# nv-tlabs/LION

Measured on AMD Instinct MI355X. Metric: shapes/sec @1000-step DDIM, Bx2048pts, higher is better.
Workload: dtype f32 (operands of the 3x3x3 voxel convolutions and of the long 1x1 convolutions cut into fp16 hi/lo pairs on the 16-bi...

## Files before the change

### lion_amd/csrc/pwconv_split.hip

```cpp
#include "split_ops.h"

namespace {

#ifdef PWS_TIMING
__device__ unsigned long long g_pws_t[128];
#define PWS_T(i) do { if (tid == 0 && blockIdx.x == 0 && blockIdx.y == 0 && blockIdx.z == 0 && (i) < 128) g_pws_t[i] = __builtin_readcyclecounter(); } while (0)
#else
#define PWS_T(i) do { } while (0)
#endif

template <int CB, int VB, bool PRO, bool STATS, int NR>
__global__ __launch_bounds__(256, 2) void pwconv_split_kernel(const float *__restrict__ x, const u4 *__restrict__ wp,
                                                           const float *__restrict__ wtail,
                                                           const float *__restrict__ bias, float *__restrict__ y,
                                                           int Cin, int Cpad, int CoutY, int L,
                                                           const float *__restrict__ pro_a,
                                                           const float *__restrict__ pro_b, float *__restrict__ stats) {
  constexpr int COT = 32 * CB, WPL = 4 * COT;
  constexpr int NDMA = WPL / 64, DMIN = NDMA / 4;
  extern __shared__ __attribute__((aligned(16))) unsigned char smem[];
  constexpr int D = NR - 1;
  u4 *sw = reinterpret_cast<u4 *>(smem);
  const int nchunks = (Cin + KS - 1) / KS;
  constexpr int RING_U4 = NR * WPL > 4 * 32 * 9 ? NR * WPL : 4 * 32 * 9;
  float *spa = reinterpret_cast<float *>(sw + RING_U4);
  float *spb = spa + (PRO ? nchunks * KS : 0);
  float *sbias = spb + (PRO ? nchunks * KS : 0);
  float *sred = sbias + COT;
  const int tid = threadIdx.x, lane = tid & 63, wave = __builtin_amdgcn_readfirstlane(tid >> 6);
  const int l32 = lane & 31, kh = lane >> 5;
  const int b = blockIdx.z, co0 = blockIdx.y * COT;
  PWS_T(0);
  if (PRO) {
    for (int c = tid; c < nchunks * KS; c += 256) {
      spa[c] = c < Cin ? pro_a[(size_t)b * Cin + c] : 0.f;
      spb[c] = c < Cin ? pro_b[(size_t)b * Cin + c] : 0.f;
    }
  }
  if (tid < COT) sbias[tid] = (bias && co0 + tid < CoutY) ? bias[co0 + tid] : 0.f;
  int colc[VB];
  bool cok[VB];
#pragma unroll
  for (int vb = 0; vb < VB; ++vb) {
    const int col = ((blockIdx.x * 4 + wave) * VB + vb) * 32 + l32;
    cok[vb] = col < L;
    colc[vb] = cok[vb] ? col : L - 1;
  }
  const __amdgpu_buffer_rsrc_t xrs = __builtin_amdgcn_make_buffer_rsrc(
      const_cast<float *>(x + (size_t)b * Cin * L), 0, Cin * L * 4, 0x00020000);
  typedef __attribute__((address_space(3))) unsigned char lds_byte;
  const uint32_t sw_lds = (uint32_t)(uintptr_t)(lds_byte *)reinterpret_cast<unsigned char *>(sw);
  auto weights_dma = [&](int q) {
    if (q >= nchunks) return;
    const uint32_t dst0 = sw_lds + (uint32_t)((q % NR) * WPL * 16);
    for (int i = wave; i < NDMA; i += 4) {
      const int e = i * 64 + lane;
      const u4 *gp = wp + ((size_t)q * 4 + e / COT) * Cpad + co0 + e % COT;
      const uint32_t dst = __builtin_amdgcn_readfirstlane(dst0 + (uint32_t)(i * 1024));
      unsigned keep;
      asm volatile("s_mov_b32 %0, m0\n\ts_mov_b32 m0, %2\n\ts_nop 0\n\tglobal_load_lds_dwordx4 %1, off\n\ts_mov_b32 m0, %0"
                   : "=&s"(keep) : "v"(gp), "s"(dst) : "memory");
    }
  };
  auto issue_x = [&](int q, float (&v)[VB][8]) {
#pragma unroll
    for (int vb = 0; vb < VB; ++vb) {
      const int off0 = ((q * KS + kh * 8) * L + colc[vb]) * 4;
#pragma unroll
      for (int j = 0; j < 8; ++j)
        v[vb][j] = __builtin_bit_cast(float, __builtin_amdgcn_raw_buffer_load_b32(xrs, off0 + j * L * 4, 0, 0));
    }
  };
  f32x16 acc[CB][VB], cor[CB][VB];
#pragma unroll
  for (int cb = 0; cb < CB; ++cb)
#pragma unroll
    for (int vb = 0; vb < VB; ++vb)
#pragma unroll
      for (int i = 0; i < 16; ++i) acc[cb][vb][i] = cor[cb][vb][i] = 0.f;
  int E[VB];
#pragma unroll
  for (int vb = 0; vb < VB; ++vb) E[vb] = 127;

  auto chunk = [&](int q, float (&v)[VB][8], float (&vnext)[VB][8]) {
    static_assert((D - 1) * (DMIN + 8 * VB) <= 63, "vmcnt is a 6-bit counter");
    const int behind = max(0, min(D - 1, nchunks - 1 - q));
    if (behind >= 3 && D > 3) wait_vm<(D - 1) * 8 * VB + (D > 3 ? 3 : 0) * DMIN>();
    else if (behind == 2 && D > 2) wait_vm<(D - 1) * 8 * VB + (D > 2 ? 2 : 0) * DMIN>();
    else if (behind == 1 && D > 1) wait_vm<(D - 1) * 8 * VB + DMIN>();
    else wait_vm<(D - 1) * 8 * VB>();
    PWS_T(2 + 4 * q);
    __syncthreads();
    PWS_T(3 + 4 * q);
    weights_dma(q + D);
    issue_x(q + D, vnext);
    PWS_T(4 + 4 * q);
    if (q >= nchunks) return;
    const u4 *swq = sw + (q % NR) * WPL;
    u4 wh[CB], wl[CB];
#pragma unroll
    for (int cb = 0; cb < CB; ++cb) { wh[cb] = swq[(0 + kh) * COT + cb * 32 + l32]; wl[cb] = swq[(2 + kh) * COT + cb * 32 + l32]; }
    u4 xh[VB], xl[VB];
#pragma unroll
    for (int vb = 0; vb < VB; ++vb) {
      float t[8];
      unsigned m = 0u;
      float pa[8], pb[8];
      if (PRO) {
        const float4 a0 = *reinterpret_cast<const float4 *>(spa + q * KS + kh * 8), a1 = *reinterpret_cast<const float4 *>(spa + q * KS + kh * 8 + 4);
        const float4 b0 = *reinterpret_cast<const float4 *>(spb + q * KS + kh * 8), b1 = *reinterpret_cast<const float4 *>(spb + q * KS + kh * 8 + 4);
        pa[0] = a0.x; pa[1] = a0.y; pa[2] = a0.z; pa[3] = a0.w; pa[4] = a1.x; pa[5] = a1.y; pa[6] = a1.z; pa[7] = a1.w;
        pb[0] = b0.x; pb[1] = b0.y; pb[2] = b0.z; pb[3] = b0.w; pb[4] = b1.x; pb[5] = b1.y; pb[6] = b1.z; pb[7] = b1.w;
      }
#pragma unroll
      for (int j = 0; j < 8; ++j) {
        float u = v[vb][j];
        if (PRO) u = pro_act(u, pa[j], pb[j]);
        u = (q * KS + kh * 8 + j < Cin && cok[vb]) ? u : 0.f;
        t[j] = u;
        const unsigned a = __float_as_uint(u) & 0x7fffffffu;
        m = (a > m && a <= 0x7f7fffffu) ? a : m;
      }
      const unsigned mo = __shfl_xor(m, 32, 64);
      m = mo > m ? mo : m;
      if (m) {
        const int e = scale_exp(__uint_as_float(m));
        if (e < E[vb]) {
          if (E[vb] != 127) {
            const float f = pow2f(max(e - PW_SPLIT_HEADROOM - E[vb], -126));
#pragma unroll
            for (int cb = 0; cb < CB; ++cb)
#pragma unroll
              for (int i = 0; i < 16; ++i) { acc[cb][vb][i] *= f; cor[cb][vb][i] *= f; }
          }
          E[vb] = e - PW_SPLIT_HEADROOM;
        }
      }
      const float xs = E[vb] == 127 ? 1.0f : pow2f(E[vb]);
#pragma unroll
      for (int k = 0; k < 4; ++k) { unsigned h2, l2; cut2(t[2 * k] * xs, t[2 * k + 1] * xs, h2, l2); xh[vb][k] = h2; xl[vb][k] = l2; }
    }
    PWS_T(64 + q);
#pragma unroll
    for (int cb = 0; cb < CB; ++cb)
#pragma unroll
      for (int vb = 0; vb < VB; ++vb) acc[cb][vb] = mma(wh[cb], xh[vb], acc[cb][vb]);
#pragma unroll
    for (int cb = 0; cb < CB; ++cb)
#pragma unroll
      for (int vb = 0; vb < VB; ++vb) cor[cb][vb] = mma(wh[cb], xl[vb], cor[cb][vb]);
#pragma unroll
    for (int cb = 0; cb < CB; ++cb)
#pragma unroll
      for (int vb = 0; vb < VB; ++vb) cor[cb][vb] = mma(wl[cb], xh[vb], cor[cb][vb]);
    PWS_T(5 + 4 * q);
  };

  static_assert(D >= 1 && D <= 4, "the wait above distinguishes up to 3 chunks in flight behind the awaited one");
  float ring[NR][VB][8];
#pragma unroll
  for (int p = 0; p < D; ++p) { weights_dma(p); issue_x(p, ring[p]); }
  PWS_T(1);
  for (int q0 = 0; q0 < nchunks; q0 += NR) {
#pragma unroll
    for (int p = 0; p < NR; ++p)
      chunk(q0 + p, ring[p], ring[(p + D) % NR]);
  }

  PWS_T(100);
  const float us_w = wtail[2];
  float *yb = y + ((size_t)b * CoutY + co0) * L;
  const bool full = co0 + COT <= CoutY;
#pragma unroll
  for (int vb = 0; vb < VB; ++vb) {
    const float us_x = E[vb] == 127 ? 1.0f : pow2f(-E[vb]);
#pragma unroll
    for (int cb = 0; cb < CB; ++cb)
#pragma unroll
      for (int i = 0; i < 16; ++i) {
        const int co = cb * 32 + (i & 3) + 8 * (i >> 2) + 4 * kh;
        const float o = ((acc[cb][vb][i] + cor[cb][vb][i] * (1.f / 2048.f)) * us_x) * us_w + sbias[co];
        acc[cb][vb][i] = cok[vb] ? o : 0.f;
      }
    float *yc = yb + colc[vb];
    if (full) {
      if (cok[vb]) {
#pragma unroll
        for (int cb = 0; cb < CB; ++cb)
#pragma unroll
          for (int i = 0; i < 16; ++i) yc[(size_t)(cb * 32 + (i & 3) + 8 * (i >> 2) + 4 * kh) * L] = acc[cb][vb][i];
      }
    } else {
#pragma unroll
      for (int cb = 0; cb < CB; ++cb)
#pragma unroll
        for (int i = 0; i < 16; ++i) {
          const int co = cb * 32 + (i & 3) + 8 * (i >> 2) + 4 * kh;
          if (cok[vb] && co0 + co < CoutY) yc[(size_t)co * L] = acc[cb][vb][i];
        }
    }
  }
  PWS_T(102);
  if (STATS) {
    __syncthreads();
    float *T = reinterpret_cast<float *>(sw) + wave * (32 * 36);
    const int hc = lane >> 5;
#pragma unroll
    for (int cb = 0; cb < CB; ++cb) {
      float s1 = 0.f, s2 = 0.f;
#pragma unroll
      for (int vb = 0; vb < VB; ++vb) {
#pragma unroll
        for (int i = 0; i < 16; ++i) T[((i & 3) + 8 * (i >> 2) + 4 * kh) * 36 + l32] = acc[cb][vb][i];
        __builtin_amdgcn_fence(__ATOMIC_RELEASE, "wavefront");
        __builtin_amdgcn_wave_barrier();
        __builtin_amdgcn_fence(__ATOMIC_ACQUIRE, "wavefront");
#pragma unroll
        for (int j = 0; j < 4; ++j) {
          const float4 t = *reinterpret_cast<const float4 *>(T + l32 * 36 + hc * 16 + 4 * j);
          s1 += t.x; s2 += t.x * t.x;
          s1 += t.y; s2 += t.y * t.y;
          s1 += t.z; s2 += t.z * t.z;
          s1 += t.w; s2 += t.w * t.w;
        }
        __builtin_amdgcn_fence(__ATOMIC_RELEASE, "wavefront");
        __builtin_amdgcn_wave_barrier();
      }
      sred[((wave * 2 + hc) * COT + cb * 32 + l32) * 2] = s1;
      sred[((wave * 2 + hc) * COT + cb * 32 + l32) * 2 + 1] = s2;
    }
    PWS_T(103);
    __syncthreads();
    for (int c = tid; c < COT && co0 + c < CoutY; c += 256) {
      float s1 = 0.f, s2 = 0.f;
#pragma unroll
      for (int w = 0; w < 8; ++w) { s1 += sred[(w * COT + c) * 2]; s2 += sred[(w * COT + c) * 2 + 1]; }
      float *o = stats + (((size_t)b * CoutY + co0 + c) * gridDim.x + blockIdx.x) * 2;
      o[0] = s1;
      o[1] = s2;
    }
  }
  PWS_T(101);
}

template <bool TR>
__global__ void pw_split_pack_kernel(const float *__restrict__ w, int Cout, int Cpad, int Cin, int nchunks,
                                     unsigned short *__restrict__ wp, unsigned *__restrict__ tail,
                                     const unsigned *__restrict__ tail_src) {
  const int i = blockIdx.x * blockDim.x + threadIdx.x;
  int ew;
  if (TR) {
    ew = (int)tail_src[1];
    if (i < 4) tail[i] = tail_src[i];
  } else {
    ew = split_tail_scale(tail, i == 0);
  }
  if (i >= nchunks * KS * Cpad) return;
  const int co = i % Cpad, k = i / Cpad, q = k / KS, g = (k % KS) / 8, j = k % 8;
  unsigned short hi = 0, lo = 0;
  if (co < Cout && k < Cin) cut((TR ? w[(size_t)k * Cout + co] : w[(size_t)co * Cin + k]) * pow2f(ew), hi, lo);
  const size_t base = (size_t)q * 4;
  wp[((base + 0 + g) * Cpad + co) * 8 + j] = hi;
  wp[((base + 2 + g) * Cpad + co) * 8 + j] = lo;
}

#ifndef PWS_NR
#define PWS_NR 5
#endif
struct PwSplitPlan { int cb, vb; };
static int pws_pad(int Cout) { return (Cout + 31) / 32 * 32; }
static PwSplitPlan pws_plan(int Cout) {
  const int blocks = pws_pad(Cout) / 32;
  if (blocks <= 0) return {0, 0};
  if (blocks % 4 == 0) return {4, 1};
  if (blocks % 2 == 0) return {2, 2};
  return {1, 2};
}
static size_t pws_halfs(int Cout, int Cin) { return (size_t)((Cin + KS - 1) / KS) * 4 * pws_pad(Cout) * 8; }

template <int CB, int VB, int NR>
static int launch_pws(const float *x, const u4 *wp, const float *wtail, const float *bias, float *y, int B, int Cin,
                      int Cout, int L, const float *pa, const float *pb, float *stats, hipStream_t st) {
  const int Cpad = pws_pad(Cout), nchunks = (Cin + KS - 1) / KS;
  const dim3 grid(lion_cdiv(L, 4 * VB * 32), Cpad / (CB * 32), B);
  const size_t ring = (size_t)NR * 4 * CB * 32 * 16, tile = (size_t)4 * 32 * 36 * 4;
  const size_t lds = (ring > tile ? ring : tile) + (size_t)((pa ? 2 * nchunks * KS : 0) + CB * 32 + 8 * CB * 32 * 2) * 4;
#define LION_PWS_GO(PRO_, ST_)                                                                             \
  {                                                                                                        \
    static LionLdsLimit cfg = {};                                                                          \
    if (int e = lion_dynamic_lds(&pwconv_split_kernel<CB, VB, PRO_, ST_, NR>, lds, cfg)) return e;             \
    pwconv_split_kernel<CB, VB, PRO_, ST_, NR><<<grid, 256, lds, st>>>(x, wp, wtail, bias, y, Cin, Cpad, Cout, L, pa, pb, stats); \
  }
  if (pa && stats) LION_PWS_GO(true, true)
  else if (pa) LION_PWS_GO(true, false)
  else if (stats) LION_PWS_GO(false, true)
  else LION_PWS_GO(false, false)
#undef LION_PWS_GO
  LION_LAUNCH_CHECK();
  return 0;
}

}

extern "C" {

#ifdef PWS_TIMING
int lion_debug_pws_times(unsigned long long *host128) {
  return hipMemcpyFromSymbol(host128, HIP_SYMBOL(g_pws_t), 1024) == hipSuccess ? 0 : -1;
}
#endif

size_t lion_pwconv_split_packed_halfs(int Cout, int Cin) { return pws_halfs(Cout, Cin) + 8; }

int lion_pwconv_split_pack_weights(const float *w, int Cout, int Cin, uint16_t *wp, lionStream_t stream) {
  if (!w || !wp || Cout <= 0 || Cin <= 0) return LION_EINVAL;
  if ((((uintptr_t)wp) & 15) != 0) return LION_EUNSUPPORTED;
  hipStream_t st = static_cast<hipStream_t>(stream);
  unsigned *tail = reinterpret_cast<unsigned *>(wp + pws_halfs(Cout, Cin));
  const int n = Cout * Cin, nchunks = (Cin + KS - 1) / KS, Cpad = pws_pad(Cout);
  if (hipMemsetAsync(tail, 0, 16, st) != hipSuccess) return LION_EINVAL;
  split_wmax_kernel<<<min(lion_cdiv(n, 2048), 128), 256, 0, st>>>(w, n, tail);
  pw_split_pack_kernel<false><<<lion_cdiv(nchunks * KS * Cpad, 256), 256, 0, st>>>(w, Cout, Cpad, Cin, nchunks, wp, tail, nullptr);
  LION_LAUNCH_CHECK();
  return 0;
}

int lion_pwconv_split_pack_weights_t(const float *w, int Cout, int Cin, const uint16_t *wp, uint16_t *wpt, lionStream_t stream) {
  if (!w || !wp || !wpt || Cout <= 0 || Cin <= 0) return LION_EINVAL;
  if (((((uintptr_t)wp) | ((uintptr_t)wpt)) & 15) != 0) return LION_EUNSUPPORTED;
  hipStream_t st = static_cast<hipStream_t>(stream);
  const unsigned *tail_src = reinterpret_cast<const unsigned *>(wp + pws_halfs(Cout, Cin));
  unsigned *tail = reinterpret_cast<unsigned *>(wpt + pws_halfs(Cin, Cout));
  const int nchunks = (Cout + KS - 1) / KS, Cpad = pws_pad(Cin);
  pw_split_pack_kernel<true><<<lion_cdiv(nchunks * KS * Cpad, 256), 256, 0, st>>>(w, Cin, Cpad, Cout, nchunks, wpt, tail, tail_src);
  LION_LAUNCH_CHECK();
  return 0;
}

int lion_pwconv_split_stat_tiles(int Cout, int Cin, int L) {
  const PwSplitPlan p = pws_plan(Cout);
  return (p.cb && Cin > 0 && L > 0) ? lion_cdiv(L, 4 * p.vb * 32) : 0;
}

int lion_pwconv_split_forward(const float *x, const uint16_t *wp, const float *bias, int B, int Cin, int Cout, int L,
                              const float *pro_a, const float *pro_b, float *y, float *stats, lionStream_t stream) {
  if (!x || !wp || !y || B <= 0 || Cin <= 0 || Cout <= 0 || L <= 0) return LION_EINVAL;
  if ((pro_a == nullptr) != (pro_b == nullptr)) return LION_EINVAL;
  if ((long)Cin * L >= (1L << 29) || Cin > 4096) return LION_EUNSUPPORTED;
  hipStream_t st = static_cast<hipStream_t>(stream);
  const u4 *w4 = reinterpret_cast<const u4 *>(wp);
  const float *wtail = reinterpret_cast<const float *>(wp + pws_halfs(Cout, Cin));
  const PwSplitPlan p = pws_plan(Cout);
  switch (p.cb) {
  case 4: return launch_pws<4, 1, PWS_NR>(x, w4, wtail, bias, y, B, Cin, Cout, L, pro_a, pro_b, stats, st);
  case 2: return launch_pws<2, 2, PWS_NR>(x, w4, wtail, bias, y, B, Cin, Cout, L, pro_a, pro_b, stats, st);
  case 1: return launch_pws<1, 2, PWS_NR>(x, w4, wtail, bias, y, B, Cin, Cout, L, pro_a, pro_b, stats, st);
  default: return LION_EUNSUPPORTED;
  }
}

}
```

Baseline: 5.401.

## Stage activation tiles via buffer-to-LDS dwordx4 DMA and vectorize output stores

Adds a WIDE variant of the split pointwise conv, used when L is a multiple of 4 and the pointers are 16-byte aligned. In it the activation chunk is staged into the LDS ring with buffer_load_dwordx4 ... lds alongside the weights, replacing the per-thread scalar dword register loads. The output is transposed through LDS and written as float4 stores. The intent is fewer, wider memory transactions and less VGPR pressure from the register ring. In exchange the LDS footprint per slot grows and the ring depth shrinks (3 or 2 slots instead of 5), which may reduce latency hiding or occupancy.

```diff
diff --git a/lion_amd/csrc/pwconv_split.hip b/lion_amd/csrc/pwconv_split.hip
--- a/lion_amd/csrc/pwconv_split.hip
+++ b/lion_amd/csrc/pwconv_split.hip
@@ -9,7 +9,7 @@
 #define PWS_T(i) do { } while (0)
 #endif
 
-template <int CB, int VB, bool PRO, bool STATS, int NR>
+template <int CB, int VB, bool PRO, bool STATS, int NR, bool WIDE>
 __global__ __launch_bounds__(256, 2) void pwconv_split_kernel(const float *__restrict__ x, const u4 *__restrict__ wp,
                                                            const float *__restrict__ wtail,
                                                            const float *__restrict__ bias, float *__restrict__ y,
@@ -18,11 +18,14 @@
                                                            const float *__restrict__ pro_b, float *__restrict__ stats) {
   constexpr int COT = 32 * CB, WPL = 4 * COT;
   constexpr int NDMA = WPL / 64, DMIN = NDMA / 4;
+  constexpr int XROW = 128 * VB;
+  constexpr int XDMA = WIDE ? 2 * VB : 0;
+  constexpr int SLOT = WPL + (WIDE ? KS * XROW / 4 : 0);
   extern __shared__ __attribute__((aligned(16))) unsigned char smem[];
   constexpr int D = NR - 1;
   u4 *sw = reinterpret_cast<u4 *>(smem);
   const int nchunks = (Cin + KS - 1) / KS;
-  constexpr int RING_U4 = NR * WPL > 4 * 32 * 9 ? NR * WPL : 4 * 32 * 9;
+  constexpr int RING_U4 = NR * SLOT > 4 * 32 * 9 ? NR * SLOT : 4 * 32 * 9;
   float *spa = reinterpret_cast<float *>(sw + RING_U4);
   float *spb = spa + (PRO ? nchunks * KS : 0);
   float *sbias = spb + (PRO ? nchunks * KS : 0);
@@ -52,7 +55,7 @@
   const uint32_t sw_lds = (uint32_t)(uintptr_t)(lds_byte *)reinterpret_cast<unsigned char *>(sw);
   auto weights_dma = [&](int q) {
     if (q >= nchunks) return;
-    const uint32_t dst0 = sw_lds + (uint32_t)((q % NR) * WPL * 16);
+    const uint32_t dst0 = sw_lds + (uint32_t)((q % NR) * SLOT * 16);
     for (int i = wave; i < NDMA; i += 4) {
       const int e = i * 64 + lane;
       const u4 *gp = wp + ((size_t)q * 4 + e / COT) * Cpad + co0 + e % COT;
@@ -62,6 +65,27 @@
                    : "=&s"(keep) : "v"(gp), "s"(dst) : "memory");
     }
   };
+  int xoff[WIDE ? XDMA : 1];
+  if (WIDE) {
+#pragma unroll
+    for (int n = 0; n < XDMA; ++n) {
+      const int e = (wave + 4 * n) * 64 + lane;
+      xoff[n] = ((e / (XROW / 4)) * L + blockIdx.x * XROW + 4 * (e % (XROW / 4))) * 4;
+    }
+  }
+  auto x_dma = [&](int q) {
+    if (q >= nchunks) return;
+    const uint32_t dst0 = sw_lds + (uint32_t)(((q % NR) * SLOT + WPL) * 16);
+    const int qoff = q * KS * L * 4;
+#pragma unroll
+    for (int n = 0; n < XDMA; ++n) {
+      const uint32_t dst = __builtin_amdgcn_readfirstlane(dst0 + (uint32_t)((wave + 4 * n) * 1024));
+      const int off = xoff[WIDE ? n : 0] + qoff;
+      unsigned keep;
+      asm volatile("s_mov_b32 %0, m0\n\ts_mov_b32 m0, %3\n\ts_nop 2\n\tbuffer_load_dwordx4 %1, %2, 0 offen lds\n\ts_mov_b32 m0, %0"
+                   : "=&s"(keep) : "v"(off), "s"(xrs), "s"(dst) : "memory");
+    }
+  };
   auto issue_x = [&](int q, float (&v)[VB][8]) {
 #pragma unroll
     for (int vb = 0; vb < VB; ++vb) {
@@ -85,18 +109,33 @@
   auto chunk = [&](int q, float (&v)[VB][8], float (&vnext)[VB][8]) {
     static_assert((D - 1) * (DMIN + 8 * VB) <= 63, "vmcnt is a 6-bit counter");
     const int behind = max(0, min(D - 1, nchunks - 1 - q));
-    if (behind >= 3 && D > 3) wait_vm<(D - 1) * 8 * VB + (D > 3 ? 3 : 0) * DMIN>();
-    else if (behind == 2 && D > 2) wait_vm<(D - 1) * 8 * VB + (D > 2 ? 2 : 0) * DMIN>();
-    else if (behind == 1 && D > 1) wait_vm<(D - 1) * 8 * VB + DMIN>();
-    else wait_vm<(D - 1) * 8 * VB>();
+    if (WIDE) {
+      if (behind >= 3 && D > 3) wait_vm<(D > 3 ? 3 : 0) * (DMIN + XDMA)>();
+      else if (behind == 2 && D > 2) wait_vm<(D > 2 ? 2 : 0) * (DMIN + XDMA)>();
+      else if (behind == 1 && D > 1) wait_vm<DMIN + XDMA>();
+      else wait_vm<0>();
+    } else {
+      if (behind >= 3 && D > 3) wait_vm<(D - 1) * 8 * VB + (D > 3 ? 3 : 0) * DMIN>();
+      else if (behind == 2 && D > 2) wait_vm<(D - 1) * 8 * VB + (D > 2 ? 2 : 0) * DMIN>();
+      else if (behind == 1 && D > 1) wait_vm<(D - 1) * 8 * VB + DMIN>();
+      else wait_vm<(D - 1) * 8 * VB>();
+    }
     PWS_T(2 + 4 * q);
     __syncthreads();
     PWS_T(3 + 4 * q);
     weights_dma(q + D);
-    issue_x(q + D, vnext);
+    if (WIDE) x_dma(q + D);
+    else issue_x(q + D, vnext);
     PWS_T(4 + 4 * q);
     if (q >= nchunks) return;
-    const u4 *swq = sw + (q % NR) * WPL;
+    const u4 *swq = sw + (q % NR) * SLOT;
+    if (WIDE) {
+      const float *xq = reinterpret_cast<const float *>(swq + WPL) + (kh * 8) * XROW + wave * VB * 32 + l32;
+#pragma unroll
+      for (int vb = 0; vb < VB; ++vb)
+#pragma unroll
+        for (int j = 0; j < 8; ++j) v[vb][j] = xq[j * XROW + vb * 32];
+    }
     u4 wh[CB], wl[CB];
 #pragma unroll
     for (int cb = 0; cb < CB; ++cb) { wh[cb] = swq[(0 + kh) * COT + cb * 32 + l32]; wl[cb] = swq[(2 + kh) * COT + cb * 32 + l32]; }
@@ -157,14 +196,21 @@
   };
 
   static_assert(D >= 1 && D <= 4, "the wait above distinguishes up to 3 chunks in flight behind the awaited one");
-  float ring[NR][VB][8];
-#pragma unroll
-  for (int p = 0; p < D; ++p) { weights_dma(p); issue_x(p, ring[p]); }
-  PWS_T(1);
-  for (int q0 = 0; q0 < nchunks; q0 += NR) {
-#pragma unroll
-    for (int p = 0; p < NR; ++p)
-      chunk(q0 + p, ring[p], ring[(p + D) % NR]);
+  float ring[WIDE ? 1 : NR][VB][8];
+  if (WIDE) {
+#pragma unroll
+    for (int p = 0; p < D; ++p) { weights_dma(p); x_dma(p); }
+    PWS_T(1);
+    for (int q = 0; q < nchunks; ++q) chunk(q, ring[0], ring[0]);
+  } else {
+#pragma unroll
+    for (int p = 0; p < D; ++p) { weights_dma(p); issue_x(p, ring[WIDE ? 0 : p]); }
+    PWS_T(1);
+    for (int q0 = 0; q0 < nchunks; q0 += NR) {
+#pragma unroll
+      for (int p = 0; p < NR; ++p)
+        chunk(q0 + p, ring[WIDE ? 0 : p], ring[WIDE ? 0 : (p + D) % NR]);
+    }
   }
 
   PWS_T(100);
@@ -182,6 +228,7 @@
         const float o = ((acc[cb][vb][i] + cor[cb][vb][i] * (1.f / 2048.f)) * us_x) * us_w + sbias[co];
         acc[cb][vb][i] = cok[vb] ? o : 0.f;
       }
+    if (WIDE) continue;
     float *yc = yb + colc[vb];
     if (full) {
       if (cok[vb]) {
@@ -200,11 +247,12 @@
         }
     }
   }
-  PWS_T(102);
-  if (STATS) {
+  if (!WIDE) PWS_T(102);
+  if (STATS || WIDE) {
     __syncthreads();
     float *T = reinterpret_cast<float *>(sw) + wave * (32 * 36);
     const int hc = lane >> 5;
+    const int r8 = lane >> 3, c4 = 4 * (lane & 7);
 #pragma unroll
     for (int cb = 0; cb < CB; ++cb) {
       float s1 = 0.f, s2 = 0.f;
@@ -215,6 +263,16 @@
         __builtin_amdgcn_fence(__ATOMIC_RELEASE, "wavefront");
         __builtin_amdgcn_wave_barrier();
         __builtin_amdgcn_fence(__ATOMIC_ACQUIRE, "wavefront");
+        if (WIDE) {
+          const int col = ((blockIdx.x * 4 + wave) * VB + vb) * 32 + c4;
+#pragma unroll
+          for (int r = 0; r < 4; ++r) {
+            const int co = cb * 32 + r * 8 + r8;
+            const float4 t = *reinterpret_cast<const float4 *>(T + (r * 8 + r8) * 36 + c4);
+            if (col < L && (full || co0 + co < CoutY)) *reinterpret_cast<float4 *>(yb + (size_t)co * L + col) = t;
+          }
+        }
+        if (STATS)
 #pragma unroll
         for (int j = 0; j < 4; ++j) {
           const float4 t = *reinterpret_cast<const float4 *>(T + l32 * 36 + hc * 16 + 4 * j);
@@ -226,11 +284,15 @@
         __builtin_amdgcn_fence(__ATOMIC_RELEASE, "wavefront");
         __builtin_amdgcn_wave_barrier();
       }
-      sred[((wave * 2 + hc) * COT + cb * 32 + l32) * 2] = s1;
-      sred[((wave * 2 + hc) * COT + cb * 32 + l32) * 2 + 1] = s2;
-    }
+      if (STATS) {
+        sred[((wave * 2 + hc) * COT + cb * 32 + l32) * 2] = s1;
+        sred[((wave * 2 + hc) * COT + cb * 32 + l32) * 2 + 1] = s2;
+      }
+    }
+    if (WIDE) PWS_T(102);
     PWS_T(103);
-    __syncthreads();
+    if (STATS) __syncthreads();
+    if (STATS)
     for (int c = tid; c < COT && co0 + c < CoutY; c += 256) {
       float s1 = 0.f, s2 = 0.f;
 #pragma unroll
@@ -267,6 +329,15 @@
 #ifndef PWS_NR
 #define PWS_NR 5
 #endif
+#ifndef PWS_NR_W41
+#define PWS_NR_W41 3
+#endif
+#ifndef PWS_NR_W22
+#define PWS_NR_W22 2
+#endif
+#ifndef PWS_NR_W12
+#define PWS_NR_W12 2
+#endif
 struct PwSplitPlan { int cb, vb; };
 static int pws_pad(int Cout) { return (Cout + 31) / 32 * 32; }
 static PwSplitPlan pws_plan(int Cout) {
@@ -278,18 +349,18 @@
 }
 static size_t pws_halfs(int Cout, int Cin) { return (size_t)((Cin + KS - 1) / KS) * 4 * pws_pad(Cout) * 8; }
 
-template <int CB, int VB, int NR>
+template <int CB, int VB, int NR, bool WIDE>
 static int launch_pws(const float *x, const u4 *wp, const float *wtail, const float *bias, float *y, int B, int Cin,
                       int Cout, int L, const float *pa, const float *pb, float *stats, hipStream_t st) {
   const int Cpad = pws_pad(Cout), nchunks = (Cin + KS - 1) / KS;
   const dim3 grid(lion_cdiv(L, 4 * VB * 32), Cpad / (CB * 32), B);
-  const size_t ring = (size_t)NR * 4 * CB * 32 * 16, tile = (size_t)4 * 32 * 36 * 4;
+  const size_t ring = (size_t)NR * (4 * CB * 32 * 16 + (WIDE ? KS * 128 * VB * 4 : 0)), tile = (size_t)4 * 32 * 36 * 4;
   const size_t lds = (ring > tile ? ring : tile) + (size_t)((pa ? 2 * nchunks * KS : 0) + CB * 32 + 8 * CB * 32 * 2) * 4;
 #define LION_PWS_GO(PRO_, ST_)                                                                             \
   {                                                                                                        \
     static LionLdsLimit cfg = {};                                                                          \
-    if (int e = lion_dynamic_lds(&pwconv_split_kernel<CB, VB, PRO_, ST_, NR>, lds, cfg)) return e;             \
-    pwconv_split_kernel<CB, VB, PRO_, ST_, NR><<<grid, 256, lds, st>>>(x, wp, wtail, bias, y, Cin, Cpad, Cout, L, pa, pb, stats); \
+    if (int e = lion_dynamic_lds(&pwconv_split_kernel<CB, VB, PRO_, ST_, NR, WIDE>, lds, cfg)) return e;             \
+    pwconv_split_kernel<CB, VB, PRO_, ST_, NR, WIDE><<<grid, 256, lds, st>>>(x, wp, wtail, bias, y, Cin, Cpad, Cout, L, pa, pb, stats); \
   }
   if (pa && stats) LION_PWS_GO(true, true)
   else if (pa) LION_PWS_GO(true, false)
@@ -351,10 +422,19 @@
   const u4 *w4 = reinterpret_cast<const u4 *>(wp);
   const float *wtail = reinterpret_cast<const float *>(wp + pws_halfs(Cout, Cin));
   const PwSplitPlan p = pws_plan(Cout);
+  const bool wide = L % 4 == 0 && ((((uintptr_t)x) | ((uintptr_t)y)) & 15) == 0;
+  if (wide) {
+    switch (p.cb) {
+    case 4: return launch_pws<4, 1, PWS_NR_W41, true>(x, w4, wtail, bias, y, B, Cin, Cout, L, pro_a, pro_b, stats, st);
+    case 2: return launch_pws<2, 2, PWS_NR_W22, true>(x, w4, wtail, bias, y, B, Cin, Cout, L, pro_a, pro_b, stats, st);
+    case 1: return launch_pws<1, 2, PWS_NR_W12, true>(x, w4, wtail, bias, y, B, Cin, Cout, L, pro_a, pro_b, stats, st);
+    default: return LION_EUNSUPPORTED;
+    }
+  }
   switch (p.cb) {
-  case 4: return launch_pws<4, 1, PWS_NR>(x, w4, wtail, bias, y, B, Cin, Cout, L, pro_a, pro_b, stats, st);
-  case 2: return launch_pws<2, 2, PWS_NR>(x, w4, wtail, bias, y, B, Cin, Cout, L, pro_a, pro_b, stats, st);
-  case 1: return launch_pws<1, 2, PWS_NR>(x, w4, wtail, bias, y, B, Cin, Cout, L, pro_a, pro_b, stats, st);
+  case 4: return launch_pws<4, 1, PWS_NR, false>(x, w4, wtail, bias, y, B, Cin, Cout, L, pro_a, pro_b, stats, st);
+  case 2: return launch_pws<2, 2, PWS_NR, false>(x, w4, wtail, bias, y, B, Cin, Cout, L, pro_a, pro_b, stats, st);
+  case 1: return launch_pws<1, 2, PWS_NR, false>(x, w4, wtail, bias, y, B, Cin, Cout, L, pro_a, pro_b, stats, st);
   default: return LION_EUNSUPPORTED;
   }
 }
```

After: 5.511 (median of 6 runs). 1.02x the previous value.
